# wangys16/FreeSplat

Measured on AMD Instinct MI355X. Metric: rendered views/sec @ 968x1296, 1.0M Gaussians, higher is better.
Workload: dtype f32

## Files before the change

### freesplat_amd/csrc/raster_fwd.hip

```cpp
#include <stdlib.h>

#include <type_traits>

#include "fs_common.h"

namespace fs {

template <int M>
__device__ __forceinline__ uint32_t lane_xor(uint32_t v)
{
    if constexpr (M == 1) return (uint32_t)__builtin_amdgcn_mov_dpp((int)v, 0xB1, 0xF, 0xF, true);
    else if constexpr (M == 2) return (uint32_t)__builtin_amdgcn_mov_dpp((int)v, 0x4E, 0xF, 0xF, true);
    else if constexpr (M == 3) return (uint32_t)__builtin_amdgcn_mov_dpp((int)v, 0x1B, 0xF, 0xF, true);
    else if constexpr (M < 32) return (uint32_t)__builtin_amdgcn_ds_swizzle((int)v, (M << 10) | 0x1F);
    else return (uint32_t)__shfl_xor((int)v, M, 64);
}
template <int M>
__device__ __forceinline__ unsigned long long lane_xor64(unsigned long long v)
{
    const uint32_t lo = lane_xor<M>((uint32_t)v), hi = lane_xor<M>((uint32_t)(v >> 32));
    return ((unsigned long long)hi << 32) | lo;
}

template <int DEG>
// ... 581 lines not shown
                    if (x > y) { a[i] = y; a[j] = x; }
                }
            }
            __syncthreads();
        }
    }
}

template <int EPT, int TM, bool REV>
__device__ __forceinline__ void thread_exchange(unsigned long long (&k)[EPT], int t, unsigned long long* lds)
{
    constexpr int HB = TM >= 128 ? 128 : TM >= 64 ? 64 : TM >= 32 ? 32 : TM >= 16 ? 16 : TM >= 8 ? 8 : TM >= 4 ? 4 : TM >= 2 ? 2 : 1;
    const bool low = (t & HB) == 0;
    unsigned long long y[EPT];
    if constexpr (TM < 64) {
#pragma unroll
        for (int e = 0; e < EPT; ++e) y[e] = lane_xor64<TM>(k[REV ? EPT - 1 - e : e]);
    } else {
        constexpr int CH = EPT * 256 > kSortLds ? kSortLds / 256 : EPT;
#pragma unroll
        for (int e0 = 0; e0 < EPT; e0 += CH) {
            __syncthreads();
#pragma unroll
            for (int e = 0; e < CH; ++e) lds[e * 256 + t] = k[REV ? EPT - 1 - (e0 + e) : e0 + e];
            __syncthreads();
#pragma unroll
            for (int e = 0; e < CH; ++e) y[e0 + e] = lds[e * 256 + (t ^ TM)];
        }
    }
#pragma unroll
    for (int e = 0; e < EPT; ++e) {
        const unsigned long long x = k[e];
        k[e] = low ? (y[e] < x ? y[e] : x) : (y[e] > x ? y[e] : x);
    }
}

template <int EPT, int J>
struct Clean {
    static __device__ __forceinline__ void run(unsigned long long (&k)[EPT], int t, unsigned long long* lds)
    {
        if constexpr (J >= EPT) {
            thread_exchange<EPT, J / EPT, false>(k, t, lds);
        } else {
#pragma unroll
            for (int e = 0; e < EPT; ++e)
                if ((e & J) == 0) {
                    const unsigned long long a = k[e], b = k[e | J];
                    if (a > b) { k[e] = b; k[e | J] = a; }
                }
        }
        if constexpr (J > 1) Clean<EPT, J / 2>::run(k, t, lds);
    }
};
template <int EPT, int K>
struct Stages {
    static __device__ __forceinline__ void run(unsigned long long (&k)[EPT], int t, unsigned long long* lds)
    {
        if constexpr (K > 2) Stages<EPT, K / 2>::run(k, t, lds);
        if constexpr (K <= EPT) {
#pragma unroll
            for (int e = 0; e < EPT; ++e) {
                const int p = e ^ (K - 1);
                if (e < p) {
                    const unsigned long long a = k[e], b = k[p];
                    if (a > b) { k[e] = b; k[p] = a; }
                }
            }
        } else {
            thread_exchange<EPT, K / EPT - 1, true>(k, t, lds);
        }
        if constexpr (K >= 4) Clean<EPT, K / 4>::run(k, t, lds);
    }
};

constexpr uint32_t kMaxBucket = 24;
template <int EPT>
__device__ __forceinline__ void sort_tile_buckets(const unsigned long long* keys, uint32_t* __restrict__ gout,
                                                  uint32_t n, unsigned long long* sk, uint32_t* cnt, uint32_t* s_red,
                                                  int tid = -1)
{
    constexpr int CAP = 256 * EPT;
    uint32_t* const list = cnt;
    const int t = tid >= 0 ? tid : (int)threadIdx.x, lane = t & 63, wave = t >> 6;
    unsigned long long k[EPT];
    uint32_t zmin = 0xFFFFFFFFu, zmax = 0u;
#pragma unroll
    for (int e = 0; e < EPT; ++e) {
        const uint32_t i = (uint32_t)(e * 256 + t);
        k[e] = i < n ? keys[i] : ~0ull;
        cnt[i] = 0u;
        if (i < n) {
            const uint32_t z = (uint32_t)(k[e] >> 32);
            zmin = min(zmin, z);
            zmax = max(zmax, z);
        }
    }
    if (t == 0) cnt[CAP] = 0u;
#pragma unroll
    for (int m = 32; m >= 1; m >>= 1) {
        zmin = min(zmin, (uint32_t)__shfl_xor((int)zmin, m, 64));
        zmax = max(zmax, (uint32_t)__shfl_xor((int)zmax, m, 64));
    }
    if (lane == 0) { s_red[wave] = zmin; s_red[4 + wave] = zmax; }
    __syncthreads();
    zmin = min(min(s_red[0], s_red[1]), min(s_red[2], s_red[3]));
    zmax = max(max(s_red[4], s_red[5]), max(s_red[6], s_red[7]));
    const float scale = (float)CAP / (float)(zmax - zmin + 1u);
    uint32_t bs[EPT];
#pragma unroll
    for (int e = 0; e < EPT; ++e) {
        const uint32_t i = (uint32_t)(e * 256 + t);
        bs[e] = 0u;
        if (i < n) {
            const uint32_t z = (uint32_t)(k[e] >> 32);
            const uint32_t b = min((uint32_t)(CAP - 1), (uint32_t)((float)(z - zmin) * scale));
            const uint32_t slot = atomicAdd(&cnt[b], 1u);
            bs[e] = (b << 8) | min(slot, 255u);
        }
    }
    __syncthreads();
    uint32_t c[EPT], sum = 0u, mx = 0u;
#pragma unroll
    for (int j = 0; j < EPT; ++j) {
        c[j] = cnt[t * EPT + j];
        sum += c[j];
        mx = max(mx, c[j]);
    }
    uint32_t inc = sum;
#pragma unroll
    for (int d = 1; d < 64; d <<= 1) {
        const uint32_t o = (uint32_t)__shfl_up((int)inc, d, 64);
        if (lane >= d) inc += o;
    }
    if (lane == 63) s_red[8 + wave] = inc;
    const bool degenerate = __syncthreads_or(mx > kMaxBucket) != 0;
    uint32_t run = inc - sum;
#pragma unroll
    for (int w = 0; w < 3; ++w) run += w < wave ? s_red[8 + w] : 0u;
    if (degenerate) {
        if constexpr ((EPT & (EPT - 1)) == 0) {
            Stages<EPT, CAP>::run(k, t, sk);
            __syncthreads();
#pragma unroll
            for (int e = 0; e < EPT; ++e) {
                const uint32_t i = (uint32_t)t * EPT + e;
                if (i < n) {
                    list[i] = (uint32_t)k[e];
                    if (gout) gout[i] = (uint32_t)k[e];
                }
            }
        } else {
            __syncthreads();
#pragma unroll
            for (int e = 0; e < EPT; ++e)
                if ((uint32_t)(e * 256 + t) < n) sk[e * 256 + t] = k[e];
            __syncthreads();
            bitonic_sort_any(sk, n);
            for (uint32_t i = (uint32_t)t; i < n; i += 256u) {
                const uint32_t wd = (uint32_t)sk[i];
                list[i] = wd;
                if (gout) gout[i] = wd;
            }
        }
        return;
    }
#pragma unroll
    for (int j = 0; j < EPT; ++j) {
        cnt[t * EPT + j] = run;
        run += c[j];
    }
    if (t == 255) cnt[CAP] = run;
    __syncthreads();
#pragma unroll
    for (int e = 0; e < EPT; ++e)
        if ((uint32_t)(e * 256 + t) < n) sk[cnt[bs[e] >> 8] + (bs[e] & 255u)] = k[e];
    __syncthreads();
    uint32_t pos[EPT];
#pragma unroll
    for (int e = 0; e < EPT; ++e) {
        pos[e] = 0u;
        if ((uint32_t)(e * 256 + t) < n) {
            const uint32_t b = bs[e] >> 8;
            const uint32_t lo = cnt[b], hi = cnt[b + 1];
            uint32_t r = 0u;
            for (uint32_t j = lo; j < hi; ++j) r += sk[j] < k[e] ? 1u : 0u;
            pos[e] = lo + r;
        }
    }
    __syncthreads();
#pragma unroll
    for (int e = 0; e < EPT; ++e) {
        if ((uint32_t)(e * 256 + t) < n) {
            list[pos[e]] = (uint32_t)k[e];
            if (gout) gout[pos[e]] = (uint32_t)k[e];
        }
    }
}

constexpr int kMaxGroups = 64;
__device__ __forceinline__ bool sort_tile_partitioned(
    const unsigned long long* __restrict__ kt, uint32_t* __restrict__ gl, uint32_t n,
                                                      unsigned long long* sk, uint32_t* cnt, uint32_t* s_red, uint32_t* s_grp)
{
    constexpr int NB = kSortLds;
    const int t = threadIdx.x, lane = t & 63, wave = t >> 6;
    uint32_t zmin = 0xFFFFFFFFu, zmax = 0u;
    for (uint32_t i = t; i < n; i += 256) {
        const uint32_t z = (uint32_t)(kt[i] >> 32);
        zmin = min(zmin, z);
        zmax = max(zmax, z);
    }
    for (int i = t; i <= NB; i += 256) cnt[i] = 0u;
#pragma unroll
    for (int m = 32; m >= 1; m >>= 1) {
        zmin = min(zmin, (uint32_t)__shfl_xor((int)zmin, m, 64));
        zmax = max(zmax, (uint32_t)__shfl_xor((int)zmax, m, 64));
    }
    if (lane == 0) { s_red[wave] = zmin; s_red[4 + wave] = zmax; }
    __syncthreads();
    zmin = min(min(s_red[0], s_red[1]), min(s_red[2], s_red[3]));
    zmax = max(max(s_red[4], s_red[5]), max(s_red[6], s_red[7]));
    const float scale = (float)NB / (float)(zmax - zmin + 1u);
    auto bin_of = [&](unsigned long long key) { return min((uint32_t)(NB - 1), (uint32_t)((float)((uint32_t)(key >> 32) - zmin) * scale)); };
    for (uint32_t i = t; i < n; i += 256) atomicAdd(&cnt[bin_of(kt[i])], 1u);
    __syncthreads();
    constexpr int BPT = NB / 256;
    uint32_t c[BPT], sum = 0u;
#pragma unroll
    for (int j = 0; j < BPT; ++j) { c[j] = cnt[t * BPT + j]; sum += c[j]; }
    uint32_t inc = sum;
#pragma unroll
    for (int d = 1; d < 64; d <<= 1) {
        const uint32_t o = (uint32_t)__shfl_up((int)inc, d, 64);
        if (lane >= d) inc += o;
    }
    if (lane == 63) s_red[8 + wave] = inc;
    __syncthreads();
    uint32_t run = inc - sum;
#pragma unroll
    for (int w = 0; w < 3; ++w) run += w < wave ? s_red[8 + w] : 0u;
#pragma unroll
    for (int j = 0; j < BPT; ++j) { cnt[t * BPT + j] = run; run += c[j]; }
    if (t == 255) cnt[NB] = run;
    __syncthreads();
    if (t == 0) {
        uint32_t g = 0, b = 0;
        bool ok = true;
        while (b < (uint32_t)NB && ok) {
            const uint32_t base = cnt[b];
            uint32_t lo = b, hi = NB;
            while (lo < hi) {
                const uint32_t mid = (lo + hi + 1) >> 1;
                if (cnt[mid] - base <= (uint32_t)kSortLds) lo = mid; else hi = mid - 1;
            }
            if (lo == b || g >= (uint32_t)kMaxGroups) { ok = false; break; }
            s_grp[g] = b;
            s_grp[kMaxGroups + 1 + g] = base;
            ++g;
            b = lo;
        }
        s_grp[g] = NB;
        s_grp[kMaxGroups + 1 + g] = n;
        s_grp[2 * kMaxGroups + 2] = ok ? g : 0xFFFFFFFFu;
    }
    __syncthreads();
    const uint32_t G = s_grp[2 * kMaxGroups + 2];
    if (G == 0xFFFFFFFFu) return false;
    for (uint32_t g = 0; g < G; ++g) {
        const uint32_t b0 = s_grp[g], b1 = s_grp[g + 1], off = s_grp[kMaxGroups + 1 + g], m = s_grp[kMaxGroups + 2 + g] - off;
        if (m == 0u) continue;
        if (t == 0) s_red[12] = 0u;
        __syncthreads();
        for (uint32_t i0 = 0; i0 < n; i0 += 256) {
            const uint32_t i = i0 + t;
            unsigned long long key = 0ull;
            bool in = false;
            if (i < n) {
                key = kt[i];
                const uint32_t b = bin_of(key);
                in = b >= b0 && b < b1;
            }
            const unsigned long long mask = __builtin_amdgcn_ballot_w64(in);
            if (mask != 0ull) {
                uint32_t base = 0u;
                if (lane == 0) base = atomicAdd(&s_red[12], (uint32_t)__popcll(mask));
                base = (uint32_t)__builtin_amdgcn_readfirstlane((int)base);
                if (in) sk[base + __builtin_amdgcn_mbcnt_hi((uint32_t)(mask >> 32), __builtin_amdgcn_mbcnt_lo((uint32_t)mask, 0u))] = key;
            }
        }
        __syncthreads();
        if (s_red[12] != m) return false;
        int tt = t;
        asm volatile("" : "+v"(tt));
        sort_tile_buckets<kSortLds / 256>(sk, gl + off, m, sk, cnt, s_red, tt);
        __syncthreads();
    }
    return true;
}

constexpr int kPairQuads = 6;
constexpr int kPairArea = 34 * kPairQuads;
template <bool FAST_EXP, bool TRACK, bool LDS_LIST>
__device__ __forceinline__ void blend_quadrant(const uint32_t* pl, int n, const float4* __restrict__ rec, float4* const cp,
                                               int H, int W, int tx, int ty, int wave, const float* __restrict__ bg,
                                               float* __restrict__ out_color, float* __restrict__ out_depth,
                                               float* __restrict__ out_alpha, float* __restrict__ final_T,
                                               int32_t* __restrict__ n_contrib)
{
    const int lane = threadIdx.x & 63;
    const int px = tx * kTile + (wave & 1) * 8 + (lane & 7);
    const int py = ty * kTile + (wave >> 1) * 8 + (lane >> 3);
    const bool inside = px < W && py < H;
    const f32x2 pfx = splat2((float)px), pfy = splat2((float)py);
    const uint32_t qbit = 1u << wave;

    float T_ = 1.0f;
    f32x2 C01 = splat2(0.0f), C2D = splat2(0.0f);
    int last = 0;
    unsigned long long done_m = __builtin_amdgcn_ballot_w64(!inside);

#define FS_BLEND_ONE(VM, AL, OM, KR, POS)                                                           \
    {                                                                                               \
        const float test_T = T_ * (OM);                                                             \
        const unsigned long long vis = (VM) & ~done_m;                                              \
        const unsigned long long okc = __builtin_amdgcn_ballot_w64(test_T >= 0.0001f);              \
        done_m |= vis & ~okc;                      \
        const bool ok = __builtin_amdgcn_inverse_ballot_w64(vis & okc);                             \
        const f32x2 wgt = splat2(ok ? (AL) * T_ : 0.0f);  \
        C01 = fma2((f32x2){(KR).x, (KR).y}, wgt, C01);                                              \
        C2D = fma2((f32x2){(KR).z, (KR).w}, wgt, C2D);                                              \
        T_ = ok ? test_T : T_;                                                                      \
        if constexpr (TRACK) last = ok ? __float_as_int(POS) : last;                                \
    }
    auto step = [&](const float4* q, auto partial, int left) __attribute__((always_inline)) {
        constexpr bool PARTIAL = decltype(partial)::value;
        const float4 c0 = q[0], c1 = q[1], c2 = q[2], c3 = q[3];
        const float4 e0 = q[6], e1 = q[7], e2 = q[8], e3 = q[9];
        const f32x2 dx = (f32x2){c0.x, c0.y} - pfx, dy = (f32x2){c0.z, c0.w} - pfy;
        const f32x2 ex = (f32x2){e0.x, e0.y} - pfx, ey = (f32x2){e0.z, e0.w} - pfy;
        const f32x2 pw = fma2((f32x2){c1.x, c1.y} * dx, dx, dy * fma2((f32x2){c1.z, c1.w}, dy, (f32x2){c2.x, c2.y} * dx));
        const f32x2 pv = fma2((f32x2){e1.x, e1.y} * ex, ex, ey * fma2((f32x2){e1.z, e1.w}, ey, (f32x2){e2.x, e2.y} * ex));
        unsigned long long ma = __builtin_amdgcn_ballot_w64(__float_as_uint(pw.x) <= __float_as_uint(c2.z));
        unsigned long long mb = __builtin_amdgcn_ballot_w64(__float_as_uint(pw.y) <= __float_as_uint(c2.w));
        unsigned long long mc = __builtin_amdgcn_ballot_w64(__float_as_uint(pv.x) <= __float_as_uint(e2.z));
        unsigned long long md = __builtin_amdgcn_ballot_w64(__float_as_uint(pv.y) <= __float_as_uint(e2.w));
        if constexpr (PARTIAL) { mb = left > 1 ? mb : 0ull; mc = left > 2 ? mc : 0ull; md = 0ull; }
        if ((((ma | mb) | (mc | md)) & ~done_m) == 0ull) return;
        const float4 ka = q[4], kb = q[5], kc = q[10], kd = q[11];
        f32x2 ew = blend_exp_of_neg<FAST_EXP>(pw), ev = blend_exp_of_neg<FAST_EXP>(pv);
        f32x2 ow = (f32x2){c3.x, c3.y} * ew, ov = (f32x2){e3.x, e3.y} * ev;
        f32x2 aw = (f32x2){fminf(0.99f, ow.x), fminf(0.99f, ow.y)};
        f32x2 av = (f32x2){fminf(0.99f, ov.x), fminf(0.99f, ov.y)};
        unsigned long long ga, gb, gc, gd;
        if constexpr (FAST_EXP) {
            const float glo = alpha_guard_lo(), ghi = alpha_guard_hi();
            ga = __builtin_amdgcn_ballot_w64(aw.x >= ghi); gb = __builtin_amdgcn_ballot_w64(aw.y >= ghi);
            gc = __builtin_amdgcn_ballot_w64(av.x >= ghi); gd = __builtin_amdgcn_ballot_w64(av.y >= ghi);
            const unsigned long long nb = (__builtin_amdgcn_ballot_w64(aw.x >= glo) & ~ga) | (__builtin_amdgcn_ballot_w64(aw.y >= glo) & ~gb)
                                        | (__builtin_amdgcn_ballot_w64(av.x >= glo) & ~gc) | (__builtin_amdgcn_ballot_w64(av.y >= glo) & ~gd);
            if (__builtin_expect(nb != 0ull, 0)) {
                ew = blend_exp_of_neg<false>(pw); ev = blend_exp_of_neg<false>(pv);
                ow = (f32x2){c3.x, c3.y} * ew; ov = (f32x2){e3.x, e3.y} * ev;
                aw = (f32x2){fminf(0.99f, ow.x), fminf(0.99f, ow.y)};
                av = (f32x2){fminf(0.99f, ov.x), fminf(0.99f, ov.y)};
                ga = __builtin_amdgcn_ballot_w64(aw.x >= 1.0f / 255.0f); gb = __builtin_amdgcn_ballot_w64(aw.y >= 1.0f / 255.0f);
                gc = __builtin_amdgcn_ballot_w64(av.x >= 1.0f / 255.0f); gd = __builtin_amdgcn_ballot_w64(av.y >= 1.0f / 255.0f);
            }
        } else {
            ga = __builtin_amdgcn_ballot_w64(aw.x >= 1.0f / 255.0f); gb = __builtin_amdgcn_ballot_w64(aw.y >= 1.0f / 255.0f);
            gc = __builtin_amdgcn_ballot_w64(av.x >= 1.0f / 255.0f); gd = __builtin_amdgcn_ballot_w64(av.y >= 1.0f / 255.0f);
        }
        const f32x2 mw = splat2(1.0f) - aw, mv = splat2(1.0f) - av;
        FS_BLEND_ONE(ma & ga, aw.x, mw.x, ka, c3.z)
        FS_BLEND_ONE(mb & gb, aw.y, mw.y, kb, c3.w)
        FS_BLEND_ONE(mc & gc, av.x, mv.x, kc, e3.z)
        if constexpr (!PARTIAL) FS_BLEND_ONE(md & gd, av.y, mv.y, kd, e3.w)
    };

    uint32_t w_cur = lane < n ? pl[lane] : 0u;
    uint32_t w_nxt = 64 + lane < n ? pl[64 + lane] : 0u;
    float4 r0 = {}, r1 = {}, r2 = {};
    if (w_cur & qbit) {
        const float4* q = rec + 3 * (size_t)(w_cur >> 4);
        r0 = q[0]; r1 = q[1]; r2 = q[2];
    }
    int rem = 0;
    for (int c = 0; c < n; c += 64) {
        if (done_m == ~0ull) break;
        const bool hit = (w_cur & qbit) != 0;
        const unsigned long long hits = __ballot(hit);
        const float4 a0 = r0, a1 = r1, a2 = r2;
        w_cur = w_nxt;
        w_nxt = c + 128 + lane < n ? pl[c + 128 + lane] : 0u;
        if (w_cur & qbit) {
            const float4* q = rec + 3 * (size_t)(w_cur >> 4);
            r0 = q[0]; r1 = q[1]; r2 = q[2];
        }
        if (!hits) continue;
        if (hit) {
            const int k = rem + __builtin_amdgcn_mbcnt_hi((uint32_t)(hits >> 32), __builtin_amdgcn_mbcnt_lo((uint32_t)hits, 0));
            float* d = (float*)(cp + (k >> 1) * kPairQuads) + (k & 1);
            d[0] = a0.x; d[2] = a0.y;
            d[4] = -a0.z; d[6] = -a0.w;
            d[8] = -a1.x; d[10] = skip_bits(a1.z);
            d[12] = a1.y; d[14] = __int_as_float(c + lane + 1);
            cp[(k >> 1) * kPairQuads + 4 + (k & 1)] = make_float4(a2.x, a2.y, a2.z, a1.w);
        }
        wave_lds_sync();
        const int total = rem + __popcll(hits), nfull = total >> 2;
        for (int p = 0; p < nfull; ++p) step(cp + 2 * p * kPairQuads, std::false_type{}, 4);
        rem = total & 3;
        if (rem != 0 && nfull != 0) {
            float4 t = {};
            if (lane < 2 * kPairQuads) t = cp[2 * nfull * kPairQuads + lane];
            if (lane < 2 * kPairQuads) cp[lane] = t;
        }
        wave_lds_sync();
    }
    if (rem != 0 && done_m != ~0ull) {
        if (lane >= rem && lane < 4) cp[(lane >> 1) * kPairQuads + 4 + (lane & 1)] = make_float4(0.0f, 0.0f, 0.0f, 0.0f);
        wave_lds_sync();
        step(cp, std::true_type{}, rem);
    }
#undef FS_BLEND_ONE
    if (inside) {
        const size_t pix = (size_t)py * W + px, HW = (size_t)H * W;
        final_T[pix] = T_;
        if constexpr (TRACK) n_contrib[pix] = last;
        out_color[pix] = fmaf(T_, bg[0], C01.x);
        out_color[HW + pix] = fmaf(T_, bg[1], C01.y);
        out_color[2 * HW + pix] = fmaf(T_, bg[2], C2D.x);
        out_depth[pix] = C2D.y;
        out_alpha[pix] = 1.0f - T_;
    }
}

static_assert(4 * kPairArea * sizeof(float4) <= kSortLds * sizeof(unsigned long long), "compaction areas must fit the key staging");
template <bool FAST_EXP, bool TRACK>
#ifndef FS_BLEND_WAVES
#define FS_BLEND_WAVES 7
#endif
__global__ __launch_bounds__(256) __attribute__((amdgpu_waves_per_eu(FS_BLEND_WAVES, FS_BLEND_WAVES))) void sort_blend_kernel(
    int H, int W, const uint32_t* __restrict__ counts, const uint32_t* __restrict__ offsets, uint32_t tile_cap,
    unsigned long long* __restrict__ keys, uint32_t* __restrict__ point_list, const float4* __restrict__ rec,
    const float* __restrict__ bg, const uint32_t* __restrict__ counters,
    float* __restrict__ out_color, float* __restrict__ out_depth, float* __restrict__ out_alpha,
    float* __restrict__ final_T, int32_t* __restrict__ n_contrib)
{
    __shared__ __attribute__((aligned(16))) unsigned long long sk[kSortLds];
    __shared__ uint32_t s_cnt[kSortLds + 1];
    __shared__ uint32_t s_red[16];
    __shared__ uint32_t s_grp[2 * kMaxGroups + 3];
    if (counters[1]) return;
    const int gx = (W + kTile - 1) / kTile, gy = (H + kTile - 1) / kTile;
    const int tile = tile_for_block(blockIdx.x, gx, gy);
    if (tile < 0) return;
    FS_PT(2, 0);
    const uint32_t n = counts[tile];
    unsigned long long* const kt = keys + (size_t)tile * tile_cap;
    uint32_t* const gl = point_list + offsets[tile];
    const bool in_lds = n <= (uint32_t)kSortLds;
    if (n == 0) {
    } else if (n <= 256u) {
        sort_tile_buckets<1>(kt, TRACK ? gl : nullptr, n, sk, s_cnt, s_red);
    } else if (n <= 512u) {
        sort_tile_buckets<2>(kt, TRACK ? gl : nullptr, n, sk, s_cnt, s_red);
    } else if (n <= 1024u) {
        sort_tile_buckets<4>(kt, TRACK ? gl : nullptr, n, sk, s_cnt, s_red);
    } else if (n <= (uint32_t)kSortLds) {
        sort_tile_buckets<kSortLds / 256>(kt, TRACK ? gl : nullptr, n, sk, s_cnt, s_red);
    }
    else if (!sort_tile_partitioned(kt, gl, n, sk, s_cnt, s_red, s_grp)) {
        __syncthreads();
        bitonic_sort_any(kt, n);
        for (uint32_t k = threadIdx.x; k < n; k += 256) gl[k] = (uint32_t)kt[k];
    }
    if (!in_lds) __threadfence_block();
    FS_PT(2, 1);
    __syncthreads();
    FS_PT(2, 2);
    const int wave = threadIdx.x >> 6;
    float4* const cp = (float4*)sk + wave * kPairArea;
    const int tx = tile % gx, ty = tile / gx;
    if (in_lds)
        blend_quadrant<FAST_EXP, TRACK, true>(s_cnt, (int)n, rec, cp, H, W, tx, ty, wave, bg, out_color, out_depth, out_alpha,
                                              final_T, n_contrib);
    else
        blend_quadrant<FAST_EXP, TRACK, false>(gl, (int)n, rec, cp, H, W, tx, ty, wave, bg, out_color, out_depth, out_alpha,
                                               final_T, n_contrib);
    FS_PT(2, 3);
}

}

using namespace fs;

FS_API int fs_raster_buffer_sizes(int32_t N, int32_t H, int32_t W, int64_t cap, size_t out[4])
{
    if (N < 0 || H <= 0 || W <= 0 || cap < 0 || !out) return FS_ERR_INVALID_ARG;
    const size_t T = (size_t)num_tiles(H, W), P = (size_t)H * W;
    out[0] = geom_bytes(N > 0 ? N : 1);
    out[1] = binning_offsets_bytes(H, W) + align_up((size_t)(cap > 0 ? cap : 1) * 4, 256);
    out[2] = align_up(P * 4, 256) * 2;
    out[3] = align_up(T * 4, 256) + align_up(T * (size_t)tile_capacity(cap, (int)T) * 8, 256);
    return FS_OK;
}

FS_API const uint32_t* fs_raster_tile_ranges(const void* binning, int32_t, int32_t)
{
    return (const uint32_t*)binning;
}
FS_API const uint32_t* fs_raster_point_list(const void* binning, int32_t H, int32_t W)
{
    return (const uint32_t*)((const char*)binning + binning_offsets_bytes(H, W));
}
FS_API const float* fs_raster_geom_records(const void* geom) { return (const float*)geom; }
FS_API const float* fs_raster_final_T(const void* image) { return (const float*)image; }
FS_API const int32_t* fs_raster_n_contrib(const void* image, int32_t H, int32_t W)
{
    return (const int32_t*)((const char*)image + align_up((size_t)H * W * 4, 256));
}

namespace fs {
constexpr int kMaxViewsInFlight = 16;
static int raster_batch()
{
    static const int n = [] {
        const char* e = getenv("FREESPLAT_RASTER_BATCH");
        const int x = e ? atoi(e) : 16;
        return x < 1 ? 1 : (x > kMaxViewsInFlight ? kMaxViewsInFlight : x);
    }();
    return n;
}

static int check_forward_args(const fs_raster_dims& d, const float* means3D, const float* cov3D, const float* shs,
                              const float* colors_precomp, const float* opacities, const int32_t* radii, int64_t cap)
{
    if (d.N < 0 || d.H <= 0 || d.W <= 0 || cap < 1) return FS_ERR_INVALID_ARG;
    if ((d.flags & FS_RASTER_SCALE_ROT) && (d.flags & FS_RASTER_COV_FULL)) return FS_ERR_INVALID_ARG;
    if (d.N > 0) {
        if (!means3D || !cov3D || !opacities || !radii) return FS_ERR_INVALID_ARG;
        if ((shs == nullptr) == (colors_precomp == nullptr)) return FS_ERR_INVALID_ARG;
    }
    if (shs && (d.sh_degree < 0 || d.sh_degree > 3 || (d.sh_degree + 1) * (d.sh_degree + 1) > d.M))
        return FS_ERR_UNSUPPORTED;
    const int gx = (d.W + kTile - 1) / kTile, gy = (d.H + kTile - 1) / kTile;
    if (gx > 32767 || gy > 32767) return FS_ERR_UNSUPPORTED;
    if (d.N > (1 << 28)) return FS_ERR_UNSUPPORTED;
    if (cap > 0xFFFFFFFFll) return FS_ERR_UNSUPPORTED;
    return FS_OK;
}

static int launch_binning(const fs_raster_dims& d, int nv, const float* means3D, const float* cov3D, const float* shs,
                          const float* colors_precomp, const float* opacities, const float* viewmatrix,
                          const float* projmatrix, const float* campos, const float* tanfov, const float* scale,
                          void* geom, size_t geom_stride, void* binning, size_t binning_stride, void* scratch,
                          size_t scratch_stride, int64_t cap, int32_t* radii, uint32_t* counters, hipStream_t st)
{
    const int T = num_tiles(d.H, d.W);
    const uint32_t tile_cap = tile_capacity(cap, T);
    hipLaunchKernelGGL(zero_counts_kernel, dim3((T + 255) / 256, nv), dim3(256), 0, st, (char*)scratch, scratch_stride, T);
    FS_CHECK_LAUNCH("zero tile counts");
    if (d.N > 0) {
        const int M = shs ? d.M : 0;
        ViewBuffers vb;
        vb.geom = (char*)geom; vb.geom_stride = geom_stride;
        vb.scratch = (char*)scratch; vb.scratch_stride = scratch_stride;
        vb.radii = radii;
        const int ch = nv >= 4 ? 1 : (nv == 2 ? 2 : 4);
        const size_t lds = (size_t)(64 * ch * M * 3) * sizeof(float) + (size_t)4 * kWaveBins * sizeof(uint32_t)
                           + (size_t)(10 * 64 * ch) * sizeof(float);
        const dim3 grid((d.N + 64 * ch - 1) / (64 * ch));
        ScopedStage prof_(kStPreprocess, st, nv);
#define FS_LAUNCH_PRE(CH, SR)                                                                                        \
        hipLaunchKernelGGL((preprocess_views_kernel<CH, SR>), grid, dim3(256), lds, st, d, nv, means3D, cov3D, shs,  \
                           colors_precomp, opacities, viewmatrix, projmatrix, campos, tanfov, scale, vb, tile_cap)
        if (d.flags & FS_RASTER_SCALE_ROT) {
            if (ch == 1) FS_LAUNCH_PRE(1, true); else if (ch == 2) FS_LAUNCH_PRE(2, true); else FS_LAUNCH_PRE(4, true);
        } else {
            if (ch == 1) FS_LAUNCH_PRE(1, false); else if (ch == 2) FS_LAUNCH_PRE(2, false); else FS_LAUNCH_PRE(4, false);
        }
#undef FS_LAUNCH_PRE
    }
    FS_CHECK_LAUNCH("preprocess_views");
    {
        ScopedStage prof_(kStTileScan, st, nv);
        hipLaunchKernelGGL(tile_scan_kernel, dim3(nv), dim3(1024), 0, st, (const char*)scratch, scratch_stride,
                           (char*)binning, binning_stride, T, counters, (unsigned long long)cap, tile_cap);
    }
    FS_CHECK_LAUNCH("tile_scan");
    return FS_OK;
}

static int launch_blend(const fs_raster_dims& d, const float* bg, void* geom, void* binning, void* image, void* scratch,
                        int64_t cap, float* out_color, float* out_depth, float* out_alpha, const uint32_t* counters,
                        hipStream_t st)
{
    const int gx = (d.W + kTile - 1) / kTile, gy = (d.H + kTile - 1) / kTile;
    const int T = gx * gy;
    const size_t P = (size_t)d.H * d.W;
    const GeomView g = geom_view(geom, d.N > 0 ? d.N : 1);
    uint32_t* offsets = (uint32_t*)binning;
    uint32_t* point_list = (uint32_t*)((char*)binning + binning_offsets_bytes(d.H, d.W));
    float* final_T = (float*)image;
    int32_t* n_contrib = (int32_t*)((char*)image + align_up(P * 4, 256));
    uint32_t* counts = (uint32_t*)scratch;
    unsigned long long* keys = (unsigned long long*)((char*)scratch + align_up((size_t)T * 4, 256));
    const uint32_t tile_cap = tile_capacity(cap, T);
    const int nblk = tile_grid_blocks(gx, gy);
    {
        ScopedStage prof_(kStRender, st);
#define FS_LAUNCH_RENDER(F, TR)                                                                                     \
        hipLaunchKernelGGL((sort_blend_kernel<F, TR>), dim3(nblk), dim3(256), 0, st, d.H, d.W, counts, offsets, tile_cap, \
                           keys, point_list, g.rec, bg, counters, out_color, out_depth, out_alpha, final_T, n_contrib)
        const bool track = !(d.flags & FS_RASTER_NO_BACKWARD_STATE);
        if (d.flags & FS_RASTER_FAST_EXP) { if (track) FS_LAUNCH_RENDER(true, true); else FS_LAUNCH_RENDER(true, false); }
        else { if (track) FS_LAUNCH_RENDER(false, true); else FS_LAUNCH_RENDER(false, false); }
#undef FS_LAUNCH_RENDER
    }
    FS_CHECK_LAUNCH("sort_blend");
    return FS_OK;
}

__global__ __launch_bounds__(256) void cov3d_from_scale_rot_kernel(int N, const float* __restrict__ rows,
                                                                   float* __restrict__ cov)
{
    for (int i = blockIdx.x * 256 + threadIdx.x; i < N; i += gridDim.x * 256) {
        float row[7], c[6];
#pragma unroll
        for (int k = 0; k < 7; ++k) row[k] = rows[7 * (size_t)i + k];
        cov_from_scale_rot(row, c);
#pragma unroll
        for (int k = 0; k < 6; ++k) cov[6 * (size_t)i + k] = c[k];
    }
}
}

FS_API int fs_raster_cov3d_from_scale_rot(int32_t N, const float* rows7, float* cov6_out, void* stream_)
{
    if (N < 0) return FS_ERR_INVALID_ARG;
    if (N == 0) return FS_OK;
    if (!rows7 || !cov6_out) return FS_ERR_INVALID_ARG;
    const int nb = (N + 255) / 256;
    const unsigned blocks = (unsigned)(nb < 8192 ? nb : 8192);
    hipLaunchKernelGGL(fs::cov3d_from_scale_rot_kernel, dim3(blocks), dim3(256), 0, (hipStream_t)stream_, N, rows7, cov6_out);
    FS_CHECK_LAUNCH("cov3d_from_scale_rot");
    return FS_OK;
}

FS_API int fs_raster_forward(const fs_raster_dims* dims, const float* means3D, const float* cov3D,
                             const float* shs, const float* colors_precomp, const float* opacities,
                             const float* bg, const float* viewmatrix, const float* projmatrix,
                             const float* campos, const float* tanfov_dev, const float* scale_dev,
                             void* geom, void* binning, void* image, void* scratch, int64_t cap, float* out_color, float* out_depth,
                             float* out_alpha, int32_t* radii, uint32_t* counters, void* stream_)
{
    if (!dims || !bg || !viewmatrix || !projmatrix || !campos || !geom || !binning || !image ||
        !scratch || !out_color || !out_depth || !out_alpha || !counters)
        return FS_ERR_INVALID_ARG;
    const fs_raster_dims d = *dims;
    int rc = check_forward_args(d, means3D, cov3D, shs, colors_precomp, opacities, radii, cap);
    if (rc != FS_OK) return rc;
    hipStream_t st = (hipStream_t)stream_;
    rc = launch_binning(d, 1, means3D, cov3D, shs, colors_precomp, opacities, viewmatrix, projmatrix, campos, tanfov_dev,
                        scale_dev, geom, 0, binning, 0, scratch, 0, cap, radii, counters, st);
    if (rc != FS_OK) return rc;
    return launch_blend(d, bg, geom, binning, image, scratch, cap, out_color, out_depth, out_alpha, counters, st);
}

namespace fs {
constexpr int kMaxStreams = 8;
struct ForkJoin {
    hipEvent_t ready = nullptr, done[kMaxStreams] = {}, batch[kMaxViewsInFlight] = {};
    bool ok = false;
    ForkJoin()
    {
        ok = hipEventCreateWithFlags(&ready, hipEventDisableTiming) == hipSuccess;
        for (int i = 0; i < kMaxStreams && ok; ++i) ok = hipEventCreateWithFlags(&done[i], hipEventDisableTiming) == hipSuccess;
        for (int i = 0; i < kMaxViewsInFlight && ok; ++i) ok = hipEventCreateWithFlags(&batch[i], hipEventDisableTiming) == hipSuccess;
    }
};
}

FS_API int fs_raster_scratch_slots(int32_t v, int32_t n_streams)
{
    if (v < 0 || n_streams < 0) return FS_ERR_INVALID_ARG;
    return v < 1 ? 1 : (v < fs::kMaxViewsInFlight ? v : fs::kMaxViewsInFlight);
}

FS_API int fs_raster_forward_views(const fs_raster_dims* dims, int32_t v, const float* means3D, const float* cov3D,
                                   const float* shs, const float* colors_precomp, const float* opacities,
                                   const float* bg, const float* viewmatrix, const float* projmatrix,
                                   const float* campos, const float* tanfov, const float* scale, void* geom,
                                   void* binning, void* image, void* scratch, const size_t strides[4], int64_t cap,
                                   float* out_color, float* out_depth, float* out_alpha, int32_t* radii,
                                   uint32_t* counters, int32_t n_streams, void* const* streams, void* main_stream)
{
    if (!dims || v < 0 || !strides || n_streams < 0 || n_streams > fs::kMaxStreams || (n_streams > 0 && !streams))
        return FS_ERR_INVALID_ARG;
    if (v == 0) return FS_OK;
    if (!bg || !viewmatrix || !projmatrix || !campos || !geom || !binning || !image || !scratch || !out_color ||
        !out_depth || !out_alpha || !counters)
        return FS_ERR_INVALID_ARG;
    const fs_raster_dims d = *dims;
    int rc = check_forward_args(d, means3D, cov3D, shs, colors_precomp, opacities, radii, cap);
    if (rc != FS_OK) return rc;
    static thread_local fs::ForkJoin* fj_dev[64] = {};
    int dev_ = 0;
    if (hipGetDevice(&dev_) != hipSuccess || dev_ < 0 || dev_ >= 64) { set_last_error("hipGetDevice", hipGetLastError()); return FS_ERR_LAUNCH; }
    if (!fj_dev[dev_]) fj_dev[dev_] = new fs::ForkJoin();
    fs::ForkJoin& fj = *fj_dev[dev_];
    const int ns = n_streams <= 1 ? 0 : (n_streams < v ? n_streams : v);
    hipStream_t main = (hipStream_t)main_stream;
    if (ns > 0 && !fj.ok) { set_last_error("event create", hipGetLastError()); return FS_ERR_LAUNCH; }
    const size_t P = (size_t)d.H * d.W;
    auto join = [&]() -> int {
        for (int s = 0; s < ns; ++s)
            if (hipEventRecord(fj.done[s], (hipStream_t)streams[s]) != hipSuccess ||
                hipStreamWaitEvent(main, fj.done[s], 0) != hipSuccess) {
                set_last_error("stream join", hipGetLastError());
                return FS_ERR_LAUNCH;
            }
        return FS_OK;
    };
    auto blend = [&](int i, void* scratch_i, hipStream_t st) {
        return fs::launch_blend(d, bg + 3 * (size_t)i, (char*)geom + strides[0] * i, (char*)binning + strides[1] * i,
                                (char*)image + strides[2] * i, scratch_i, cap, out_color + 3 * P * i, out_depth + P * i,
                                out_alpha + P * i, counters + 2 * (size_t)i, st);
    };
    const int VB = fs::raster_batch();
    for (int c0 = 0; c0 < v && rc == FS_OK; c0 += fs::kMaxViewsInFlight) {
        const int c1 = c0 + fs::kMaxViewsInFlight < v ? c0 + fs::kMaxViewsInFlight : v;
        for (int b0 = c0, k = 0; b0 < c1 && rc == FS_OK; b0 += VB, ++k) {
            const int nb = b0 + VB < c1 ? VB : c1 - b0;
            char* const scratch_b = (char*)scratch + strides[3] * (size_t)(b0 - c0);
            rc = fs::launch_binning(d, nb, means3D, cov3D, shs, colors_precomp, opacities, viewmatrix + 16 * (size_t)b0,
                                    projmatrix + 16 * (size_t)b0, campos + 3 * (size_t)b0,
                                    tanfov ? tanfov + 2 * (size_t)b0 : nullptr, scale ? scale + b0 : nullptr,
                                    (char*)geom + strides[0] * b0, strides[0], (char*)binning + strides[1] * b0, strides[1],
                                    scratch_b, strides[3], cap, radii ? radii + (size_t)d.N * b0 : nullptr,
                                    counters + 2 * (size_t)b0, main);
            if (rc != FS_OK) break;
            if (ns > 0 && hipEventRecord(fj.batch[k], main) != hipSuccess) { set_last_error("event record", hipGetLastError()); rc = FS_ERR_LAUNCH; break; }
            for (int i = b0; i < b0 + nb && rc == FS_OK; ++i) {
                hipStream_t st = ns > 0 ? (hipStream_t)streams[i % ns] : main;
                if (ns > 0 && hipStreamWaitEvent(st, fj.batch[k], 0) != hipSuccess) { set_last_error("stream wait", hipGetLastError()); rc = FS_ERR_LAUNCH; break; }
                rc = blend(i, scratch_b + strides[3] * (size_t)(i - b0), st);
            }
        }
        const int jr = join();
        if (rc == FS_OK) rc = jr;
    }
    return rc;
}

#ifdef FS_PHASE_TRACE
FS_API int fs_debug_phase_trace(unsigned long long* dst)
{
    static unsigned long long z[fs::kPtKernels * fs::kPtBlocks * fs::kPtSlots];
    if (hipMemcpyFromSymbol(dst, HIP_SYMBOL(fs::g_phase_trace), sizeof(z)) != hipSuccess) return FS_ERR_LAUNCH;
    return hipMemcpyToSymbol(HIP_SYMBOL(fs::g_phase_trace), z, sizeof(z)) == hipSuccess ? FS_OK : FS_ERR_LAUNCH;
}
#endif
```

Before: 4406.

## Queue hit indices per wave so gaussian record loads are dense and prefetched

Instead of each lane loading a gaussian record for its own list slot (sparse, many lanes idle when few hits), each wave compacts the indices of hits for its quadrant into a 64-entry LDS queue. It then loads 64 records at once with all lanes active, and the fill for the next batch overlaps with blending the current one. This cuts wasted memory fetches on sparse hit patterns and adds LDS queue traffic, extra syncs and more complex control flow. It also makes the wave index uniform via readfirstlane and adds early exit inside the step loop.

```diff
diff --git a/freesplat_amd/csrc/raster_fwd.hip b/freesplat_amd/csrc/raster_fwd.hip
--- a/freesplat_amd/csrc/raster_fwd.hip
+++ b/freesplat_amd/csrc/raster_fwd.hip
@@ -907,6 +907,7 @@
 constexpr int kPairArea = 34 * kPairQuads;
 template <bool FAST_EXP, bool TRACK, bool LDS_LIST>
 __device__ __forceinline__ void blend_quadrant(const uint32_t* pl, int n, const float4* __restrict__ rec, float4* const cp,
+                                               uint32_t* const qi, uint32_t* const qw,
                                                int H, int W, int tx, int ty, int wave, const float* __restrict__ bg,
                                                float* __restrict__ out_color, float* __restrict__ out_depth,
                                                float* __restrict__ out_alpha, float* __restrict__ final_T,
@@ -985,42 +986,82 @@
     uint32_t w_cur = lane < n ? pl[lane] : 0u;
     uint32_t w_nxt = 64 + lane < n ? pl[64 + lane] : 0u;
     float4 r0 = {}, r1 = {}, r2 = {};
-    if (w_cur & qbit) {
-        const float4* q = rec + 3 * (size_t)(w_cur >> 4);
-        r0 = q[0]; r1 = q[1]; r2 = q[2];
-    }
-    int rem = 0;
-    for (int c = 0; c < n; c += 64) {
+    int r_pos = 0;
+    int c = 0;
+    int filled = 0;
+    auto take = [&](int cnt) __attribute__((always_inline)) {
+        wave_lds_sync();
+        if (lane < cnt) {
+            const uint32_t e = qi[lane];
+            uint32_t w;
+            if constexpr (LDS_LIST) w = pl[e]; else w = qw[lane];
+            const float4* q = rec + 3 * (size_t)(w >> 4);
+            r0 = q[0]; r1 = q[1]; r2 = q[2];
+            if constexpr (TRACK) r_pos = (int)e + 1;
+        }
+    };
+    auto next_batch = [&]() __attribute__((always_inline)) -> int {
+        while (c < n) {
+            const bool hit = (w_cur & qbit) != 0;
+            const unsigned long long hits = __ballot(hit);
+            const uint32_t w_hit = w_cur;
+            const uint32_t e = (uint32_t)(c + lane);
+            w_cur = w_nxt;
+            w_nxt = c + 128 + lane < n ? pl[c + 128 + lane] : 0u;
+            c += 64;
+            if (!hits) continue;
+            const int slot = filled + __builtin_amdgcn_mbcnt_hi((uint32_t)(hits >> 32), __builtin_amdgcn_mbcnt_lo((uint32_t)hits, 0));
+            if (hit && slot < 64) {
+                qi[slot] = e;
+                if constexpr (!LDS_LIST) qw[slot] = w_hit;
+            }
+            filled += __popcll(hits);
+            if (filled >= 64) {
+                take(64);
+                if (hit && slot >= 64) {
+                    qi[slot - 64] = e;
+                    if constexpr (!LDS_LIST) qw[slot - 64] = w_hit;
+                }
+                filled -= 64;
+                return 64;
+            }
+        }
+        const int cnt = filled;
+        if (cnt != 0) take(cnt);
+        filled = 0;
+        return cnt;
+    };
+    int rem = 0, cur = 0;
+    for (;;) {
         if (done_m == ~0ull) break;
-        const bool hit = (w_cur & qbit) != 0;
-        const unsigned long long hits = __ballot(hit);
-        const float4 a0 = r0, a1 = r1, a2 = r2;
-        w_cur = w_nxt;
-        w_nxt = c + 128 + lane < n ? pl[c + 128 + lane] : 0u;
-        if (w_cur & qbit) {
-            const float4* q = rec + 3 * (size_t)(w_cur >> 4);
-            r0 = q[0]; r1 = q[1]; r2 = q[2];
-        }
-        if (!hits) continue;
-        if (hit) {
-            const int k = rem + __builtin_amdgcn_mbcnt_hi((uint32_t)(hits >> 32), __builtin_amdgcn_mbcnt_lo((uint32_t)hits, 0));
+        if (lane < cur) {
+            const int k = rem + lane;
             float* d = (float*)(cp + (k >> 1) * kPairQuads) + (k & 1);
-            d[0] = a0.x; d[2] = a0.y;
-            d[4] = -a0.z; d[6] = -a0.w;
-            d[8] = -a1.x; d[10] = skip_bits(a1.z);
-            d[12] = a1.y; d[14] = __int_as_float(c + lane + 1);
-            cp[(k >> 1) * kPairQuads + 4 + (k & 1)] = make_float4(a2.x, a2.y, a2.z, a1.w);
-        }
-        wave_lds_sync();
-        const int total = rem + __popcll(hits), nfull = total >> 2;
-        for (int p = 0; p < nfull; ++p) step(cp + 2 * p * kPairQuads, std::false_type{}, 4);
-        rem = total & 3;
-        if (rem != 0 && nfull != 0) {
-            float4 t = {};
-            if (lane < 2 * kPairQuads) t = cp[2 * nfull * kPairQuads + lane];
-            if (lane < 2 * kPairQuads) cp[lane] = t;
-        }
-        wave_lds_sync();
+            d[0] = r0.x; d[2] = r0.y;
+            d[4] = -r0.z; d[6] = -r0.w;
+            d[8] = -r1.x; d[10] = skip_bits(r1.z);
+            d[12] = r1.y;
+            if constexpr (TRACK) d[14] = __int_as_float(r_pos);
+            cp[(k >> 1) * kPairQuads + 4 + (k & 1)] = make_float4(r2.x, r2.y, r2.z, r1.w);
+        }
+        const int nxt = next_batch();
+        if (cur != 0) {
+            wave_lds_sync();
+            const int total = rem + cur, nfull = total >> 2;
+            for (int p = 0; p < nfull; ++p) {
+                if (done_m == ~0ull) break;
+                step(cp + 2 * p * kPairQuads, std::false_type{}, 4);
+            }
+            rem = total & 3;
+            if (rem != 0 && nfull != 0) {
+                float4 t = {};
+                if (lane < 2 * kPairQuads) t = cp[2 * nfull * kPairQuads + lane];
+                if (lane < 2 * kPairQuads) cp[lane] = t;
+            }
+            wave_lds_sync();
+        }
+        cur = nxt;
+        if (cur == 0) break;
     }
     if (rem != 0 && done_m != ~0ull) {
         if (lane >= rem && lane < 4) cp[(lane >> 1) * kPairQuads + 4 + (lane & 1)] = make_float4(0.0f, 0.0f, 0.0f, 0.0f);
@@ -1029,7 +1070,9 @@
     }
 #undef FS_BLEND_ONE
     if (inside) {
-        const size_t pix = (size_t)py * W + px, HW = (size_t)H * W;
+        const int ln = __builtin_amdgcn_mbcnt_hi(~0u, __builtin_amdgcn_mbcnt_lo(~0u, 0));
+        const int ox = tx * kTile + (wave & 1) * 8 + (ln & 7), oy = ty * kTile + (wave >> 1) * 8 + (ln >> 3);
+        const size_t pix = (size_t)oy * W + ox, HW = (size_t)H * W;
         final_T[pix] = T_;
         if constexpr (TRACK) n_contrib[pix] = last;
         out_color[pix] = fmaf(T_, bg[0], C01.x);
@@ -1040,7 +1083,8 @@
     }
 }
 
-static_assert(4 * kPairArea * sizeof(float4) <= kSortLds * sizeof(unsigned long long), "compaction areas must fit the key staging");
+static_assert(4 * (kPairArea * sizeof(float4) + 64 * sizeof(uint32_t)) <= kSortLds * sizeof(unsigned long long),
+              "compaction areas and hit queues must fit the key staging");
 template <bool FAST_EXP, bool TRACK>
 #ifndef FS_BLEND_WAVES
 #define FS_BLEND_WAVES 7
@@ -1084,14 +1128,16 @@
     FS_PT(2, 1);
     __syncthreads();
     FS_PT(2, 2);
-    const int wave = threadIdx.x >> 6;
+    const int wave = __builtin_amdgcn_readfirstlane(threadIdx.x >> 6);
     float4* const cp = (float4*)sk + wave * kPairArea;
+    uint32_t* const qi = (uint32_t*)((float4*)sk + 4 * kPairArea) + wave * 64;
+    uint32_t* const qw = s_cnt + wave * 64;
     const int tx = tile % gx, ty = tile / gx;
     if (in_lds)
-        blend_quadrant<FAST_EXP, TRACK, true>(s_cnt, (int)n, rec, cp, H, W, tx, ty, wave, bg, out_color, out_depth, out_alpha,
+        blend_quadrant<FAST_EXP, TRACK, true>(s_cnt, (int)n, rec, cp, qi, nullptr, H, W, tx, ty, wave, bg, out_color, out_depth, out_alpha,
                                               final_T, n_contrib);
     else
-        blend_quadrant<FAST_EXP, TRACK, false>(gl, (int)n, rec, cp, H, W, tx, ty, wave, bg, out_color, out_depth, out_alpha,
+        blend_quadrant<FAST_EXP, TRACK, false>(gl, (int)n, rec, cp, qi, qw, H, W, tx, ty, wave, bg, out_color, out_depth, out_alpha,
                                                final_T, n_contrib);
     FS_PT(2, 3);
 }
```

After: 4517 (median of 6 runs). +2.5%, better.
